# claserken/SISS

Hardware: AMD Instinct MI355X
Metric: unlearning samples/sec (= unlearning-steps/sec x batch x gpus), CelebA-HQ-256 DDPM SISS (higher is better)
Workload: dtype bf16; 1 GPU; delete_celeb.yaml: CelebA-HQ 256x256 DDPM UNet (113.7M params), SISS lambd=0.5, t=999, bf16, bs=16/GPU, GA=1, scaling_norm=500, AdamW lr 5e-6; loss_fn=importance_sampling_with_mixture, global_batch=16, grad_accum=1, parallelism=dp1, hipgraph=True

## Files before the change

### siss_amd/csrc/common.h

```cpp
#pragma once
#include <hip/hip_runtime.h>
#include <stdint.h>

typedef uint16_t bf16_t;

typedef __attribute__((ext_vector_type(8))) short bf16x8_t;
typedef __attribute__((ext_vector_type(4))) float f32x4_t;
typedef __attribute__((ext_vector_type(16))) float f32x16_t;
typedef __attribute__((ext_vector_type(4))) uint32_t u32x4_t;
typedef __attribute__((ext_vector_type(2))) uint32_t u32x2_t;
typedef __attribute__((ext_vector_type(2))) float f32x2_t;
typedef __attribute__((ext_vector_type(2))) __bf16 bf16x2_t;

#define SISS_OK 0
#define SISS_ERR_ARG 1
#define SISS_ERR_LAUNCH 2

#define SISS_CHECK_ARG(cond) \
    do {                     \
        if (!(cond)) return SISS_ERR_ARG; \
    } while (0)

#define SISS_LAUNCH_RET()                                 \
    do {                                                  \
        return hipGetLastError() == hipSuccess ? SISS_OK : SISS_ERR_LAUNCH; \
    } while (0)

__device__ __forceinline__ float bf2f(bf16_t v) {
    return __builtin_bit_cast(float, (uint32_t)v << 16);
}
__device__ __forceinline__ bf16_t f2bf(float f) {
    __bf16 b = (__bf16)f;
    return __builtin_bit_cast(bf16_t, b);
}
__device__ __forceinline__ float bfround(float f) { return bf2f(f2bf(f)); }
__device__ __forceinline__ float to_f(bf16_t v) { return bf2f(v); }
__device__ __forceinline__ float to_f(float v) { return v; }
template <typename T> __device__ __forceinline__ T from_f(float f);
template <> __device__ __forceinline__ bf16_t from_f<bf16_t>(float f) { return f2bf(f); }
template <> __device__ __forceinline__ float from_f<float>(float f) { return f; }
__device__ __forceinline__ uint32_t pack_bf2(float lo, float hi) {
    typedef float f32x2_pk __attribute__((ext_vector_type(2)));
    typedef __bf16 bf16x2_pk __attribute__((ext_vector_type(2)));
    const bf16x2_pk b = __builtin_convertvector(f32x2_pk{lo, hi}, bf16x2_pk);
    return __builtin_bit_cast(uint32_t, b);
}

__device__ __forceinline__ uint32_t add_bf16x2(uint32_t a, uint32_t b) {
    const float lo = __builtin_bit_cast(float, a << 16) + __builtin_bit_cast(float, b << 16);
    const float hi = __builtin_bit_cast(float, a & 0xffff0000u) + __builtin_bit_cast(float, b & 0xffff0000u);
    uint32_t r;
    asm("v_cvt_pk_bf16_f32 %0, %1, %2" : "=v"(r) : "v"(lo), "v"(hi));
    return r;
}

__device__ __forceinline__ float wave_sum(float v) {
#pragma unroll
    for (int o = 32; o > 0; o >>= 1) v += __shfl_xor(v, o, 64);
    return v;
}
__device__ __forceinline__ double wave_sum_d(double v) {
#pragma unroll
    for (int o = 32; o > 0; o >>= 1) v += __shfl_xor(v, o, 64);
    return v;
}

__device__ __forceinline__ float sum_lanes_mod8(float t) {
    t += __builtin_bit_cast(float, __builtin_amdgcn_update_dpp(0, __builtin_bit_cast(int, t), 0x128 , 0xf, 0xf, false));
    unsigned u = __builtin_bit_cast(unsigned, t), u2 = u;
    asm volatile("" : "+v"(u2));
    const auto a = __builtin_amdgcn_permlane16_swap(u, u2, false, false);
    unsigned a0 = a[0], a1 = a[1];
    asm volatile("" : "+v"(a0), "+v"(a1));
    t = __builtin_bit_cast(float, a0) + __builtin_bit_cast(float, a1);
    unsigned v = __builtin_bit_cast(unsigned, t), v2 = v;
    asm volatile("" : "+v"(v2));
    const auto b = __builtin_amdgcn_permlane32_swap(v, v2, false, false);
    unsigned b0 = b[0], b1 = b[1];
    asm volatile("" : "+v"(b0), "+v"(b1));
    return __builtin_bit_cast(float, b0) + __builtin_bit_cast(float, b1);
}

__device__ __forceinline__ float sigmoid_f(float z) { return __builtin_amdgcn_rcpf(1.f + __expf(-z)); }
__device__ __forceinline__ float silu_f(float z) { return z * sigmoid_f(z); }
__device__ __forceinline__ float dsilu_f(float z) {
    const float s = sigmoid_f(z);
    return s * (1.f + z * (1.f - s));
}

__device__ __forceinline__ void gelu_parts(float g, float& Phi, float& e) {
    const float x = fabsf(g) * 0.70710678118654752f;
    const float t = __builtin_amdgcn_rcpf(fmaf(0.3275911f, x, 1.f));
    e = __builtin_amdgcn_exp2f(g * g * -0.72134752044448170f);
    const float poly = t * fmaf(t, fmaf(t, fmaf(t, fmaf(t, 1.061405429f, -1.453152027f), 1.421413741f), -0.284496736f), 0.254829592f);
    const float erf_abs = fmaf(-poly, e, 1.f);
    Phi = 0.5f * (1.f + copysignf(erf_abs, g));
}
__device__ __forceinline__ float gelu_f(float g) { float P, e; gelu_parts(g, P, e); return g * P; }
__device__ __forceinline__ float dgelu_f(float g) { float P, e; gelu_parts(g, P, e); return fmaf(g * 0.3989422804014327f, e, P); }


__device__ __forceinline__ void glds16_asm(const void* g, unsigned lds_dst) {
    unsigned keep;
    asm volatile("s_mov_b32 %0, m0\n\ts_mov_b32 m0, %2\n\ts_nop 0\n\tglobal_load_lds_dwordx4 %1, off\n\ts_mov_b32 m0, %0"
                 : "=&s"(keep) : "v"(g), "s"(lds_dst) : "memory");
}
__device__ __forceinline__ void glds16_saddr(unsigned off, const void* base, unsigned lds_dst) {
    asm volatile("s_mov_b32 m0, %1\n\ts_nop 0\n\tglobal_load_lds_dwordx4 %0, %2" :: "v"(off), "s"(lds_dst), "s"(base) : "memory");
}
__device__ __forceinline__ unsigned lds_addr(const void* p) {
    return (unsigned)(size_t)(__attribute__((address_space(3))) const char*)p;
}

static inline int cdiv(long a, long b) { return (int)((a + b - 1) / b); }

constexpr int kMaxDevices = 64;
constexpr int kQsTileRows = 254, kQsHalfRows = 128;
static inline int siss_current_device() {
    int dev = 0;
    return hipGetDevice(&dev) == hipSuccess && dev >= 0 && dev < kMaxDevices ? dev : -1;
}
static inline int siss_ensure_smem(const void* kernel, int bytes, unsigned char (&done)[kMaxDevices]) {
    const int dev = siss_current_device();
    if (dev < 0) return SISS_ERR_LAUNCH;
    if (!__atomic_load_n(&done[dev], __ATOMIC_ACQUIRE)) {
        if (hipFuncSetAttribute(kernel, hipFuncAttributeMaxDynamicSharedMemorySize, bytes) != hipSuccess) return SISS_ERR_LAUNCH;
        __atomic_store_n(&done[dev], (unsigned char)1, __ATOMIC_RELEASE);
    }
    return SISS_OK;
}

enum SissKernelId { SISS_K_NT = 0, SISS_K_NT_C3P, SISS_K_FLASH_FWD, SISS_K_FLASH_BWD, SISS_K_NT_SPLITK, SISS_K_TN1, SISS_K_TN3,
                    SISS_K_GN_SLAB, SISS_K_GN_QSTATS, SISS_K_FLASH_QSPLIT, SISS_K_ATTN1H_FWD, SISS_K_ATTN1H_BWD, SISS_K_TN_PAIR, SISS_K_FLASH32, SISS_K_FLASH32_FWD, SISS_K_NT_WIDE, SISS_K_GN_SC, SISS_K_COUNT };
void siss_count_dispatch(int kernel_id);
void* siss_workspace(long* bytes);
```

### siss_amd/csrc/lora.hip

```cpp
#include "common.h"

namespace {

constexpr int kTile = 64;

struct LoraJob {
    long w_off, a_off, b_off, w0_off;
    int O, I, ptile0, mtile0;
};

template <bool MERGE>
__device__ __forceinline__ int find_job(const LoraJob* jobs, int njobs, int tile) {
    int lo = 0, hi = njobs - 1;
    while (lo < hi) {
        const int mid = (lo + hi + 1) >> 1;
        if ((MERGE ? jobs[mid].mtile0 : jobs[mid].ptile0) <= tile) lo = mid; else hi = mid - 1;
    }
    return lo;
}

constexpr f32x4_t kZero = {0.f, 0.f, 0.f, 0.f};

__device__ __forceinline__ f32x4_t ld_k4(const float* row, int k, int len, bool ok, bool vec) {
    if (!ok || k >= len) return kZero;
    if (vec) return *reinterpret_cast<const f32x4_t*>(row + k);
    f32x4_t v = kZero;
#pragma unroll
    for (int j = 0; j < 4; ++j)
        if (k + j < len) v[j] = row[k + j];
    return v;
}

template <int NT>
__global__ __launch_bounds__(256) void lora_project_kernel(const float* __restrict__ grads, long set_stride, int nsets,
                                                           const float* __restrict__ lora_p, float* __restrict__ lora_g,
                                                           long lora_set_stride, const LoraJob* __restrict__ jobs, int njobs, int r,
                                                           float s) {
    const int tile = blockIdx.x, set = blockIdx.y;
    const LoraJob jb = jobs[find_job<false>(jobs, njobs, tile)];
    const int O = jb.O, I = jb.I, lt = tile - jb.ptile0, rb = (O + kTile - 1) / kTile;
    const int lane = threadIdx.x & 63, wv = threadIdx.x >> 6, li = lane & 15, q = lane >> 4;
    const bool live = set < nsets;
    const float* dW = grads + (long)set * set_stride + jb.w_off;
    const float* A = lora_p + jb.a_off;
    const float* B = lora_p + jb.b_off;
    f32x4_t acc[NT];
#pragma unroll
    for (int n = 0; n < NT; ++n) acc[n] = kZero;

    if (lt < rb) {
        const int o0 = lt * kTile + wv * 16;
        if (o0 >= O) return;
        if (live) {
            const bool vec = (I & 3) == 0;
            const bool rok = o0 + li < O;
            const float* wrow = dW + (long)(o0 + li) * I;
            for (int k0 = 0; k0 < I; k0 += 16) {
                const int k = k0 + 4 * q;
                const f32x4_t a = ld_k4(wrow, k, I, rok, vec);
                f32x4_t b[NT];
#pragma unroll
                for (int n = 0; n < NT; ++n) b[n] = ld_k4(A + (long)(n * 16 + li) * I, k, I, n * 16 + li < r, vec);
#pragma unroll
                for (int j = 0; j < 4; ++j)
#pragma unroll
                    for (int n = 0; n < NT; ++n) acc[n] = __builtin_amdgcn_mfma_f32_16x16x4f32(a[j], b[n][j], acc[n], 0, 0, 0);
            }
        }
        float* dB = lora_g + (long)set * lora_set_stride + jb.b_off;
#pragma unroll
        for (int n = 0; n < NT; ++n)
#pragma unroll
            for (int j = 0; j < 4; ++j) {
                const int row = o0 + 4 * q + j, col = n * 16 + li;
                if (row < O && col < r) dB[(long)row * r + col] = s * acc[n][j];
            }
    } else {
        const int i0 = (lt - rb) * kTile + wv * 16;
        if (i0 >= I) return;
        const int col = i0 + li;
        const bool cok = col < I;
        if (live) {
#pragma unroll 4
            for (int o = 0; o < O; o += 4) {
                const int ko = o + q;
                const bool kok = ko < O;
                const float bv = (kok && cok) ? dW[(long)ko * I + col] : 0.f;
#pragma unroll
                for (int m = 0; m < NT; ++m) {
                    const float av = (kok && m * 16 + li < r) ? B[(long)ko * r + m * 16 + li] : 0.f;
                    acc[m] = __builtin_amdgcn_mfma_f32_16x16x4f32(av, bv, acc[m], 0, 0, 0);
                }
            }
        }
        float* dA = lora_g + (long)set * lora_set_stride + jb.a_off;
#pragma unroll
        for (int m = 0; m < NT; ++m)
#pragma unroll
            for (int j = 0; j < 4; ++j) {
                const int row = m * 16 + 4 * q + j;
                if (row < r && cok) dA[(long)row * I + col] = s * acc[m][j];
            }
    }
}

__global__ __launch_bounds__(256) void lora_merge_kernel(float* __restrict__ flat, bf16_t* __restrict__ shadow,
                                                         const float* __restrict__ w0, const float* __restrict__ lora_p,
                                                         const LoraJob* __restrict__ jobs, int njobs, int r, float s) {
    const int tile = blockIdx.x;
    const LoraJob jb = jobs[find_job<true>(jobs, njobs, tile)];
    const int O = jb.O, I = jb.I, lt = tile - jb.mtile0, cb = (I + kTile - 1) / kTile;
    const int lane = threadIdx.x & 63, wv = threadIdx.x >> 6, li = lane & 15, q = lane >> 4;
    const int o0 = (lt / cb) * kTile + wv * 16, i0 = (lt % cb) * kTile;
    if (o0 >= O) return;
    const float* A = lora_p + jb.a_off;
    const float* B = lora_p + jb.b_off;
    f32x4_t acc[4] = {kZero, kZero, kZero, kZero};
    if (s != 0.f) {
        const bool rok = o0 + li < O;
        for (int k0 = 0; k0 < r; k0 += 4) {
            const int k = k0 + q;
            const bool kok = k < r;
            const float av = (kok && rok) ? B[(long)(o0 + li) * r + k] : 0.f;
#pragma unroll
            for (int c = 0; c < 4; ++c) {
                const int col = i0 + c * 16 + li;
                const float bv = (kok && col < I) ? A[(long)k * I + col] : 0.f;
                acc[c] = __builtin_amdgcn_mfma_f32_16x16x4f32(av, bv, acc[c], 0, 0, 0);
            }
        }
    }
#pragma unroll
    for (int c = 0; c < 4; ++c)
#pragma unroll
        for (int j = 0; j < 4; ++j) {
            const int row = o0 + 4 * q + j, col = i0 + c * 16 + li;
            if (row < O && col < I) {
                const long idx = (long)row * I + col;
                const float base = w0[jb.w0_off + idx];
                const float v = s != 0.f ? fmaf(s, acc[c][j], base) : base;
                flat[jb.w_off + idx] = v;
                if (shadow) shadow[jb.w_off + idx] = f2bf(v);
            }
        }
}

}

extern "C" {

long siss_lora_tile(void) {
    return kTile;
}

int siss_lora_project(const float* grads, long set_stride, int nsets, const float* lora_p, float* lora_g, long lora_set_stride,
                      const void* jobs, int njobs, int r, float s, int total_tiles, void* stream) {
    SISS_CHECK_ARG(grads && lora_p && lora_g && jobs && njobs >= 1 && total_tiles >= njobs);
    SISS_CHECK_ARG((nsets == 1 || nsets == 2) && r >= 1 && r <= 64 && set_stride % 4 == 0 && lora_set_stride % 4 == 0);
    SISS_CHECK_ARG(((uintptr_t)grads | (uintptr_t)lora_p | (uintptr_t)lora_g) % 16 == 0);
    const dim3 grid(total_tiles, 2), block(256);
    const LoraJob* jt = static_cast<const LoraJob*>(jobs);
    hipStream_t st = (hipStream_t)stream;
#define SISS_LORA_PROJECT(NT) \
    lora_project_kernel<NT><<<grid, block, 0, st>>>(grads, set_stride, nsets, lora_p, lora_g, lora_set_stride, jt, njobs, r, s)
    switch ((r + 15) / 16) {
        case 1: SISS_LORA_PROJECT(1); break;
        case 2: SISS_LORA_PROJECT(2); break;
        case 3: SISS_LORA_PROJECT(3); break;
        default: SISS_LORA_PROJECT(4); break;
    }
#undef SISS_LORA_PROJECT
    SISS_LAUNCH_RET();
}

int siss_lora_merge(float* flat, void* shadow, const float* w0, const float* lora_p, const void* jobs, int njobs, int r, float s,
                    int total_tiles, void* stream) {
    SISS_CHECK_ARG(flat && w0 && lora_p && jobs && njobs >= 1 && total_tiles >= njobs && r >= 1 && r <= 64);
    lora_merge_kernel<<<dim3(total_tiles), dim3(256), 0, (hipStream_t)stream>>>(flat, static_cast<bf16_t*>(shadow), w0, lora_p,
                                                                                 static_cast<const LoraJob*>(jobs), njobs, r, s);
    SISS_LAUNCH_RET();
}

}
```

### siss_amd/csrc/timeemb.hip

```cpp
#include "common.h"

namespace {

constexpr int kThreads = 256;
constexpr int kMaxM = 4096;

__global__ void sincos_kernel(const int64_t* __restrict__ t, float* __restrict__ out, int B, int dim, int flip,
                              float freq_shift) {
    const int i = blockIdx.x * blockDim.x + threadIdx.x;
    const int half = dim / 2;
    if (i >= B * half) return;
    const int b = i / half, j = i - b * half;
    const float freq = expf(-logf(10000.f) * (float)j / ((float)half - freq_shift));
    const float arg = (float)t[b] * freq;
    const float s = sinf(arg), c = cosf(arg);
    float* o = out + (long)b * dim;
    if (flip) { o[j] = c; o[half + j] = s; }
    else { o[j] = s; o[half + j] = c; }
}

__global__ __launch_bounds__(kThreads) void linear_fwd_kernel(const float* __restrict__ x,
                                                              const float* __restrict__ W,
                                                              const float* __restrict__ b, float* __restrict__ y,
                                                              int M, int N, int K, int act_in) {
    const int lane = threadIdx.x & 63;
    const int n = blockIdx.x * (kThreads / 64) + (threadIdx.x >> 6);
    if (n >= N) return;
    for (int m0 = 0; m0 < M; m0 += 8) {
        float acc[8] = {};
        for (int k = lane; k < K; k += 64) {
            const float w = W[(long)n * K + k];
#pragma unroll
            for (int i = 0; i < 8; ++i) {
                if (m0 + i < M) {
                    float xv = x[(long)(m0 + i) * K + k];
                    if (act_in) xv = silu_f(xv);
                    acc[i] += xv * w;
                }
            }
        }
#pragma unroll
        for (int i = 0; i < 8; ++i) {
            const float s = wave_sum(acc[i]);
            if (lane == 0 && m0 + i < M) y[(long)(m0 + i) * N + n] = s + b[n];
        }
    }
}

__device__ __forceinline__ float dy_eff(const float* dy, const float* yact, int m, int n, int N, int Mx) {
    float d = dy[(long)m * N + n];
    if (yact) d *= dsilu_f(yact[(long)(m % Mx) * N + n]);
    return d;
}

__global__ __launch_bounds__(256) void linear_bwd_dx_kernel(const float* __restrict__ dy, const float* __restrict__ yact,
                                                            const float* __restrict__ W, float* __restrict__ dx, int M2,
                                                            int Mx, int N, int K, int accumulate) {
    __shared__ float part[4][64];
    const int m = blockIdx.y, lane = threadIdx.x & 63, w = threadIdx.x >> 6;
    const int k = blockIdx.x * 64 + lane;
    const int n0 = (int)((long)N * w / 4), n1 = (int)((long)N * (w + 1) / 4);
    float acc = 0.f;
    if (k < K)
        for (int n = n0; n < n1; ++n) acc += dy_eff(dy, yact, m, n, N, Mx) * W[(long)n * K + k];
    part[w][lane] = acc;
    __syncthreads();
    if (w == 0 && k < K) {
        const float t = part[0][lane] + part[1][lane] + part[2][lane] + part[3][lane];
        const long i = (long)m * K + k;
        dx[i] = accumulate ? dx[i] + t : t;
    }
}

__global__ void linear_bwd_dw_kernel(const float* __restrict__ dy, const float* __restrict__ yact,
                                     const float* __restrict__ x, float* __restrict__ dW, float* __restrict__ db,
                                     float* __restrict__ db2, int M2, int Mx, int set_rows, long set_stride_w, long set_stride_b, int N,
                                     int K, int act_in) {
    const long i = (long)blockIdx.x * blockDim.x + threadIdx.x;
    const int nsets = M2 / set_rows;
    if (i >= (long)nsets * N * K) return;
    const int set = i / ((long)N * K);
    const long rem = i - (long)set * N * K;
    const int n = rem / K, k = rem - (long)n * K;
    float acc = 0.f, bsum = 0.f;
    for (int j = 0; j < set_rows; ++j) {
        const int m = set * set_rows + j;
        const float d = dy_eff(dy, yact, m, n, N, Mx);
        float xv = x[(long)(m % Mx) * K + k];
        if (act_in) xv = silu_f(xv);
        acc += d * xv;
        bsum += d;
    }
    dW[(long)set * set_stride_w + (long)n * K + k] += acc;
    if (k == 0) {
        db[(long)set * set_stride_b + n] += bsum;
        if (db2) db2[(long)set * set_stride_b + n] += bsum;
    }
}


__global__ __launch_bounds__(kThreads) void multi_fwd_kernel(const float* __restrict__ x, const float* __restrict__ P,
                                                             const long* __restrict__ woff, const long* __restrict__ boff,
                                                             float* __restrict__ y, int M, int Ntot, int K) {
    const int lane = threadIdx.x & 63;
    const int n = blockIdx.x * (kThreads / 64) + (threadIdx.x >> 6);
    if (n >= Ntot) return;
    const float* W = P + woff[n];
    for (int m0 = 0; m0 < M; m0 += 8) {
        float acc[8] = {};
        for (int k = lane; k < K; k += 64) {
            const float w = W[k];
#pragma unroll
            for (int i = 0; i < 8; ++i)
                if (m0 + i < M) acc[i] += silu_f(x[(long)(m0 + i) * K + k]) * w;
        }
#pragma unroll
        for (int i = 0; i < 8; ++i) {
            const float s = wave_sum(acc[i]);
            if (lane == 0 && m0 + i < M) y[(long)(m0 + i) * Ntot + n] = s + P[boff[n]];
        }
    }
}

constexpr int kDwCols = 32, kDwRows = 32;
__global__ __launch_bounds__(256) void multi_bwd_dw_kernel(const float* __restrict__ dy, const float* __restrict__ x, float* __restrict__ G,
                                                           const long* __restrict__ woff, const long* __restrict__ boff,
                                                           const long* __restrict__ boff2, int Mx, int set_rows, long set_stride,
                                                           int Ntot, int K) {
    __shared__ float sdy[kDwRows][kDwCols + 1];
    const int k = blockIdx.x * 256 + threadIdx.x;
    const int n0 = blockIdx.y * kDwCols, set = blockIdx.z;
    const int ncols = Ntot - n0 < kDwCols ? Ntot - n0 : kDwCols;
    float acc[kDwCols];
#pragma unroll
    for (int c = 0; c < kDwCols; ++c) acc[c] = 0.f;
    float bsum = 0.f;
    for (int j0 = 0; j0 < set_rows; j0 += kDwRows) {
        const int nr = set_rows - j0 < kDwRows ? set_rows - j0 : kDwRows;
        __syncthreads();
        for (int i = threadIdx.x; i < kDwRows * kDwCols; i += 256) {
            const int r = i / kDwCols, c = i - r * kDwCols;
            sdy[r][c] = (r < nr && c < ncols) ? dy[(long)(set * set_rows + j0 + r) * Ntot + n0 + c] : 0.f;
        }
        __syncthreads();
        if (blockIdx.x == 0 && threadIdx.x < ncols)
            for (int r = 0; r < nr; ++r) bsum += sdy[r][threadIdx.x];
        if (k < K) {
            for (int r = 0; r < nr; ++r) {
                const float sx = silu_f(x[(long)((set * set_rows + j0 + r) % Mx) * K + k]);
#pragma unroll
                for (int c = 0; c < kDwCols; ++c) acc[c] += sdy[r][c] * sx;
            }
        }
    }
    float* g = G + (long)set * set_stride;
    if (k < K) {
#pragma unroll
        for (int c = 0; c < kDwCols; ++c)
            if (c < ncols) g[woff[n0 + c] + k] += acc[c];
    }
    if (blockIdx.x == 0 && threadIdx.x < ncols) {
        g[boff[n0 + threadIdx.x]] += bsum;
        g[boff2[n0 + threadIdx.x]] += bsum;
    }
}

constexpr int kDxSplit = 512;
__global__ __launch_bounds__(256) void multi_bwd_dx_kernel(const float* __restrict__ dy, const float* __restrict__ P,
                                                           const long* __restrict__ woff, float* __restrict__ dx,
                                                           int M2, int Ntot, int K) {
    const int k = blockIdx.x * 256 + threadIdx.x;
    const int m = blockIdx.y;
    const int n0 = blockIdx.z * kDxSplit;
    const int n1 = n0 + kDxSplit < Ntot ? n0 + kDxSplit : Ntot;
    if (k >= K) return;
    const float* d = dy + (long)m * Ntot;
    float a0 = 0.f, a1 = 0.f, a2 = 0.f, a3 = 0.f;
    int n = n0;
    for (; n + 4 <= n1; n += 4) {
        a0 += d[n] * P[woff[n] + k];
        a1 += d[n + 1] * P[woff[n + 1] + k];
        a2 += d[n + 2] * P[woff[n + 2] + k];
        a3 += d[n + 3] * P[woff[n + 3] + k];
    }
    for (; n < n1; ++n) a0 += d[n] * P[woff[n] + k];
    atomicAdd(dx + (long)m * K + k, (a0 + a1) + (a2 + a3));
}

}

extern "C" {

int siss_timestep_sincos(const int64_t* t, float* out, int B, int dim, int flip_sin_to_cos, float freq_shift, void* stream) {
    SISS_CHECK_ARG(t && out && B > 0 && dim > 0 && dim % 2 == 0);
    sincos_kernel<<<cdiv((long)B * dim / 2, 128), 128, 0, (hipStream_t)stream>>>(t, out, B, dim, flip_sin_to_cos, freq_shift);
    SISS_LAUNCH_RET();
}

int siss_linear_small_fwd(const float* x, const float* W, const float* b, float* y, int M, int N, int K, int act_in_silu, void* stream) {
    SISS_CHECK_ARG(x && W && b && y && M > 0 && M <= kMaxM && N > 0 && K > 0);
    linear_fwd_kernel<<<cdiv(N, kThreads / 64), kThreads, 0, (hipStream_t)stream>>>(x, W, b, y, M, N, K, act_in_silu);
    SISS_LAUNCH_RET();
}

int siss_linear_small_bwd(const float* dy, const float* yact, const float* x, const float* W, float* dx, int accumulate_dx,
                          float* dW, float* db, float* db2, int M2, int Mx, int set_rows, long set_stride_w,
                          long set_stride_b, int N, int K, int act_in_silu, void* stream) {
    SISS_CHECK_ARG(dy && x && W && dW && db && M2 > 0 && Mx > 0 && set_rows > 0 && M2 % set_rows == 0 && N > 0 && K > 0);
    hipStream_t st = (hipStream_t)stream;
    if (dx) linear_bwd_dx_kernel<<<dim3(cdiv(K, 64), M2), 256, 0, st>>>(dy, yact, W, dx, M2, Mx, N, K, accumulate_dx);
    const long tot = (long)(M2 / set_rows) * N * K;
    linear_bwd_dw_kernel<<<cdiv(tot, 256), 256, 0, st>>>(dy, yact, x, dW, db, db2, M2, Mx, set_rows, set_stride_w, set_stride_b, N, K, act_in_silu);
    SISS_LAUNCH_RET();
}

int siss_linear_multi_fwd(const float* x, const float* params, const long* woff, const long* boff, float* y, int M,
                          int Ntot, int K, void* stream) {
    SISS_CHECK_ARG(x && params && woff && boff && y && M > 0 && M <= kMaxM && Ntot > 0 && K > 0);
    multi_fwd_kernel<<<cdiv(Ntot, kThreads / 64), kThreads, 0, (hipStream_t)stream>>>(x, params, woff, boff, y, M, Ntot, K);
    SISS_LAUNCH_RET();
}

int siss_linear_multi_bwd(const float* dy, const float* x, const float* params, float* grads, const long* woff,
                          const long* boff, const long* boff2, float* dx, int M2, int Mx, int set_rows,
                          long set_stride, int Ntot, int K, void* stream) {
    SISS_CHECK_ARG(dy && x && params && grads && woff && boff && boff2 && dx);
    SISS_CHECK_ARG(M2 > 0 && M2 <= kMaxM && Mx > 0 && set_rows > 0 && M2 % set_rows == 0 && Ntot > 0 && K > 0);
    hipStream_t st = (hipStream_t)stream;
    const dim3 gw(cdiv(K, 256), cdiv(Ntot, kDwCols), M2 / set_rows);
    multi_bwd_dw_kernel<<<gw, 256, 0, st>>>(dy, x, grads, woff, boff, boff2, Mx, set_rows, set_stride, Ntot, K);
    dim3 grid(cdiv(K, 256), M2, cdiv(Ntot, kDxSplit));
    multi_bwd_dx_kernel<<<grid, 256, 0, st>>>(dy, params, woff, dx, M2, Ntot, K);
    SISS_LAUNCH_RET();
}

}
```

Before: 313.8 samples/sec.

## Use fp32 MFMA tiles for small-linear backward dW and split-N dX

Replaces the scalar per-element dW kernels for the time-embedding linears (plain and multi-table) with one templated kernel that accumulates 16x16 tiles using fp32 MFMA, loading existing gradients into the accumulators and writing them back with vector stores. The dX backward now uses an MFMA tile kernel split along N into workspace partials, followed by a separate reduce kernel, with the old kernel kept as a fallback when the workspace is too small. The aim is to cut the cost of these many small backward GEMMs. It adds a workspace dependency and an extra launch, and changes the order of floating-point summation.

```diff
diff --git a/siss_amd/csrc/common.h b/siss_amd/csrc/common.h
--- a/siss_amd/csrc/common.h
+++ b/siss_amd/csrc/common.h
@@ -81,6 +81,16 @@
     return __builtin_bit_cast(float, b0) + __builtin_bit_cast(float, b1);
 }
 
+__device__ __forceinline__ f32x4_t ld_k4(const float* row, int k, int len, bool ok, bool vec) {
+    f32x4_t v = {0.f, 0.f, 0.f, 0.f};
+    if (!ok || k >= len) return v;
+    if (vec) return *reinterpret_cast<const f32x4_t*>(row + k);
+#pragma unroll
+    for (int j = 0; j < 4; ++j)
+        if (k + j < len) v[j] = row[k + j];
+    return v;
+}
+
 __device__ __forceinline__ float sigmoid_f(float z) { return __builtin_amdgcn_rcpf(1.f + __expf(-z)); }
 __device__ __forceinline__ float silu_f(float z) { return z * sigmoid_f(z); }
 __device__ __forceinline__ float dsilu_f(float z) {
diff --git a/siss_amd/csrc/lora.hip b/siss_amd/csrc/lora.hip
--- a/siss_amd/csrc/lora.hip
+++ b/siss_amd/csrc/lora.hip
@@ -20,16 +20,6 @@
 }
 
 constexpr f32x4_t kZero = {0.f, 0.f, 0.f, 0.f};
-
-__device__ __forceinline__ f32x4_t ld_k4(const float* row, int k, int len, bool ok, bool vec) {
-    if (!ok || k >= len) return kZero;
-    if (vec) return *reinterpret_cast<const f32x4_t*>(row + k);
-    f32x4_t v = kZero;
-#pragma unroll
-    for (int j = 0; j < 4; ++j)
-        if (k + j < len) v[j] = row[k + j];
-    return v;
-}
 
 template <int NT>
 __global__ __launch_bounds__(256) void lora_project_kernel(const float* __restrict__ grads, long set_stride, int nsets,
diff --git a/siss_amd/csrc/timeemb.hip b/siss_amd/csrc/timeemb.hip
--- a/siss_amd/csrc/timeemb.hip
+++ b/siss_amd/csrc/timeemb.hip
@@ -19,6 +19,20 @@
     else { o[j] = s; o[half + j] = c; }
 }
 
+__device__ __forceinline__ bool aligned16(const void* p) { return ((uintptr_t)p & 15) == 0; }
+
+template <bool TABLE>
+__device__ __forceinline__ const float* weight_row(const float* W, const long* woff, int n, int K) {
+    return TABLE ? W + woff[n] : W + (long)n * K;
+}
+
+template <bool FAST>
+__device__ __forceinline__ f32x4_t ld_op(const float* row, int k, int len, bool ok, bool vec) {
+    if (!FAST) return ld_k4(row, k, len, ok, vec);
+    const f32x4_t v = *reinterpret_cast<const f32x4_t*>(row + (k < len ? k : 0));
+    return ok && k < len ? v : f32x4_t{0.f, 0.f, 0.f, 0.f};
+}
+
 __global__ __launch_bounds__(kThreads) void linear_fwd_kernel(const float* __restrict__ x,
                                                               const float* __restrict__ W,
                                                               const float* __restrict__ b, float* __restrict__ y,
@@ -43,6 +57,29 @@
         for (int i = 0; i < 8; ++i) {
             const float s = wave_sum(acc[i]);
             if (lane == 0 && m0 + i < M) y[(long)(m0 + i) * N + n] = s + b[n];
+        }
+    }
+}
+
+__global__ __launch_bounds__(kThreads) void multi_fwd_kernel(const float* __restrict__ x, const float* __restrict__ P,
+                                                             const long* __restrict__ woff, const long* __restrict__ boff,
+                                                             float* __restrict__ y, int M, int Ntot, int K) {
+    const int lane = threadIdx.x & 63;
+    const int n = blockIdx.x * (kThreads / 64) + (threadIdx.x >> 6);
+    if (n >= Ntot) return;
+    const float* W = P + woff[n];
+    for (int m0 = 0; m0 < M; m0 += 8) {
+        float acc[8] = {};
+        for (int k = lane; k < K; k += 64) {
+            const float w = W[k];
+#pragma unroll
+            for (int i = 0; i < 8; ++i)
+                if (m0 + i < M) acc[i] += silu_f(x[(long)(m0 + i) * K + k]) * w;
+        }
+#pragma unroll
+        for (int i = 0; i < 8; ++i) {
+            const float s = wave_sum(acc[i]);
+            if (lane == 0 && m0 + i < M) y[(long)(m0 + i) * Ntot + n] = s + P[boff[n]];
         }
     }
 }
@@ -72,97 +109,230 @@
     }
 }
 
-__global__ void linear_bwd_dw_kernel(const float* __restrict__ dy, const float* __restrict__ yact,
-                                     const float* __restrict__ x, float* __restrict__ dW, float* __restrict__ db,
-                                     float* __restrict__ db2, int M2, int Mx, int set_rows, long set_stride_w, long set_stride_b, int N,
-                                     int K, int act_in) {
-    const long i = (long)blockIdx.x * blockDim.x + threadIdx.x;
-    const int nsets = M2 / set_rows;
-    if (i >= (long)nsets * N * K) return;
-    const int set = i / ((long)N * K);
-    const long rem = i - (long)set * N * K;
-    const int n = rem / K, k = rem - (long)n * K;
-    float acc = 0.f, bsum = 0.f;
-    for (int j = 0; j < set_rows; ++j) {
-        const int m = set * set_rows + j;
-        const float d = dy_eff(dy, yact, m, n, N, Mx);
-        float xv = x[(long)(m % Mx) * K + k];
-        if (act_in) xv = silu_f(xv);
-        acc += d * xv;
-        bsum += d;
-    }
-    dW[(long)set * set_stride_w + (long)n * K + k] += acc;
-    if (k == 0) {
-        db[(long)set * set_stride_b + n] += bsum;
-        if (db2) db2[(long)set * set_stride_b + n] += bsum;
-    }
-}
-
-
-__global__ __launch_bounds__(kThreads) void multi_fwd_kernel(const float* __restrict__ x, const float* __restrict__ P,
-                                                             const long* __restrict__ woff, const long* __restrict__ boff,
-                                                             float* __restrict__ y, int M, int Ntot, int K) {
-    const int lane = threadIdx.x & 63;
-    const int n = blockIdx.x * (kThreads / 64) + (threadIdx.x >> 6);
-    if (n >= Ntot) return;
-    const float* W = P + woff[n];
-    for (int m0 = 0; m0 < M; m0 += 8) {
-        float acc[8] = {};
-        for (int k = lane; k < K; k += 64) {
-            const float w = W[k];
-#pragma unroll
-            for (int i = 0; i < 8; ++i)
-                if (m0 + i < M) acc[i] += silu_f(x[(long)(m0 + i) * K + k]) * w;
-        }
-#pragma unroll
-        for (int i = 0; i < 8; ++i) {
-            const float s = wave_sum(acc[i]);
-            if (lane == 0 && m0 + i < M) y[(long)(m0 + i) * Ntot + n] = s + P[boff[n]];
-        }
-    }
-}
-
-constexpr int kDwCols = 32, kDwRows = 32;
-__global__ __launch_bounds__(256) void multi_bwd_dw_kernel(const float* __restrict__ dy, const float* __restrict__ x, float* __restrict__ G,
-                                                           const long* __restrict__ woff, const long* __restrict__ boff,
-                                                           const long* __restrict__ boff2, int Mx, int set_rows, long set_stride,
-                                                           int Ntot, int K) {
-    __shared__ float sdy[kDwRows][kDwCols + 1];
-    const int k = blockIdx.x * 256 + threadIdx.x;
-    const int n0 = blockIdx.y * kDwCols, set = blockIdx.z;
-    const int ncols = Ntot - n0 < kDwCols ? Ntot - n0 : kDwCols;
-    float acc[kDwCols];
-#pragma unroll
-    for (int c = 0; c < kDwCols; ++c) acc[c] = 0.f;
+constexpr int kDwSub = 4;
+template <bool TABLE>
+__global__ __launch_bounds__(256, 3) void linear_bwd_dw_tile_kernel(const float* __restrict__ dy, const float* __restrict__ yact,
+                                                                 const float* __restrict__ x, float* __restrict__ dW,
+                                                                 float* __restrict__ db, float* __restrict__ db2,
+                                                                 const long* __restrict__ woff, const long* __restrict__ boff,
+                                                                 const long* __restrict__ boff2, int Mx, int set_rows,
+                                                                 long set_stride_w, long set_stride_b, int N, int K, int act_in) {
+    const int lane = threadIdx.x & 63, wv = threadIdx.x >> 6, li = lane & 15, q = lane >> 4;
+    const int n0 = blockIdx.y * 64 + 16 * wv, set = blockIdx.z;
+    if (n0 >= N) return;
+    const int k0 = blockIdx.x * (64 * kDwSub), kl = k0 + 4 * li;
+    const bool k4 = (K & 3) == 0, xvec = k4 && aligned16(x);
+    float* grow[4];
+    bool nok[4], gal = true;
+#pragma unroll
+    for (int i = 0; i < 4; ++i) {
+        const int n = n0 + 4 * q + i;
+        nok[i] = n < N;
+        const int nc = nok[i] ? n : N - 1;
+        grow[i] = dW + (long)set * set_stride_w + (TABLE ? woff[nc] : (long)nc * K);
+        gal = gal && aligned16(grow[i]);
+    }
+    const bool gfast = k4 && __all(gal);
+    f32x4_t acc[kDwSub][4];
+    if (gfast) {
+#pragma unroll
+        for (int i = 0; i < 4; ++i)
+#pragma unroll
+            for (int t = 0; t < kDwSub; ++t) {
+                const f32x4_t g = ld_op<true>(grow[i], kl + 64 * t, K, nok[i], true);
+#pragma unroll
+                for (int c = 0; c < 4; ++c) acc[t][c][i] = g[c];
+            }
+    } else {
+#pragma unroll
+        for (int t = 0; t < kDwSub; ++t)
+#pragma unroll
+            for (int c = 0; c < 4; ++c) acc[t][c] = f32x4_t{0.f, 0.f, 0.f, 0.f};
+    }
+    const bool colok = n0 + li < N;
+    const int ncol = colok ? n0 + li : N - 1;
     float bsum = 0.f;
-    for (int j0 = 0; j0 < set_rows; j0 += kDwRows) {
-        const int nr = set_rows - j0 < kDwRows ? set_rows - j0 : kDwRows;
-        __syncthreads();
-        for (int i = threadIdx.x; i < kDwRows * kDwCols; i += 256) {
-            const int r = i / kDwCols, c = i - r * kDwCols;
-            sdy[r][c] = (r < nr && c < ncols) ? dy[(long)(set * set_rows + j0 + r) * Ntot + n0 + c] : 0.f;
-        }
-        __syncthreads();
-        if (blockIdx.x == 0 && threadIdx.x < ncols)
-            for (int r = 0; r < nr; ++r) bsum += sdy[r][threadIdx.x];
-        if (k < K) {
-            for (int r = 0; r < nr; ++r) {
-                const float sx = silu_f(x[(long)((set * set_rows + j0 + r) % Mx) * K + k]);
-#pragma unroll
-                for (int c = 0; c < kDwCols; ++c) acc[c] += sdy[r][c] * sx;
+    for (int j0 = 0; j0 < set_rows; j0 += 4) {
+        const bool jok = j0 + q < set_rows;
+        const int m = set * set_rows + (jok ? j0 + q : 0), mx = m % Mx;
+        float a = dy[(long)m * N + ncol];
+        const float ya = yact ? yact[(long)mx * N + ncol] : 0.f;
+        const float* xrow = x + (long)mx * K;
+        f32x4_t bv[kDwSub];
+        if (xvec) {
+#pragma unroll
+            for (int t = 0; t < kDwSub; ++t) bv[t] = ld_op<true>(xrow, kl + 64 * t, K, jok, true);
+        } else {
+#pragma unroll
+            for (int t = 0; t < kDwSub; ++t) bv[t] = ld_k4(xrow, kl + 64 * t, K, jok, false);
+        }
+        if (yact) a *= dsilu_f(ya);
+        if (!(jok && colok)) a = 0.f;
+        bsum += a;
+        if (act_in) {
+#pragma unroll
+            for (int t = 0; t < kDwSub; ++t)
+#pragma unroll
+                for (int c = 0; c < 4; ++c) bv[t][c] = silu_f(bv[t][c]);
+        }
+#pragma unroll
+        for (int t = 0; t < kDwSub; ++t)
+#pragma unroll
+            for (int c = 0; c < 4; ++c) acc[t][c] = __builtin_amdgcn_mfma_f32_16x16x4f32(a, bv[t][c], acc[t][c], 0, 0, 0);
+    }
+#pragma unroll
+    for (int i = 0; i < 4; ++i)
+#pragma unroll
+        for (int t = 0; t < kDwSub; ++t) {
+            const int k = kl + 64 * t;
+            if (!nok[i] || k >= K) continue;
+            if (gfast) {
+                *reinterpret_cast<f32x4_t*>(grow[i] + k) = f32x4_t{acc[t][0][i], acc[t][1][i], acc[t][2][i], acc[t][3][i]};
+            } else {
+#pragma unroll
+                for (int c = 0; c < 4; ++c)
+                    if (k + c < K) grow[i][k + c] += acc[t][c][i];
             }
         }
-    }
-    float* g = G + (long)set * set_stride;
-    if (k < K) {
-#pragma unroll
-        for (int c = 0; c < kDwCols; ++c)
-            if (c < ncols) g[woff[n0 + c] + k] += acc[c];
-    }
-    if (blockIdx.x == 0 && threadIdx.x < ncols) {
-        g[boff[n0 + threadIdx.x]] += bsum;
-        g[boff2[n0 + threadIdx.x]] += bsum;
-    }
+    if (blockIdx.x == 0) {
+        bsum += __shfl_xor(bsum, 16, 64);
+        bsum += __shfl_xor(bsum, 32, 64);
+        if (q == 0 && colok) {
+            const long sb = (long)set * set_stride_b;
+            db[sb + (TABLE ? boff[ncol] : (long)ncol)] += bsum;
+            if (db2) db2[sb + (TABLE ? boff2[ncol] : (long)ncol)] += bsum;
+        }
+    }
+}
+
+
+template <bool FAST>
+__device__ __forceinline__ void dx_operands(f32x4_t (&a)[2], f32x4_t (&ya)[2], f32x4_t (&bv)[4], const float* const (&dyrow)[2],
+                                            const float* const (&yrow)[2], const bool (&rok)[2], int nq, int N,
+                                            const float* const (&wrow)[4], const bool (&nok)[4], int kl, int K, bool dvec, bool k4) {
+#pragma unroll
+    for (int g = 0; g < 2; ++g) {
+        a[g] = ld_op<FAST>(dyrow[g], nq, N, rok[g], dvec);
+        ya[g] = ld_op<FAST>(yrow[g], nq, N, rok[g], dvec);
+    }
+#pragma unroll
+    for (int j = 0; j < 4; ++j) bv[j] = ld_op<FAST>(wrow[j], kl, K, nok[j], k4 && aligned16(wrow[j]));
+}
+
+template <bool TABLE>
+__global__ __launch_bounds__(256) void linear_bwd_dx_tile_kernel(const float* __restrict__ dy, const float* __restrict__ yact,
+                                                                 const float* __restrict__ W, const long* __restrict__ woff,
+                                                                 float* __restrict__ part, int M2, int Mx, int N, int K, int Kp,
+                                                                 int chunk) {
+    __shared__ f32x4_t red[4][2][16][16];
+    const int lane = threadIdx.x & 63, wv = threadIdx.x >> 6, li = lane & 15, q = lane >> 4;
+    const int k0 = blockIdx.x * 64, kl = k0 + 4 * li;
+    const int nb = blockIdx.y * chunk, ne = nb + chunk < N ? nb + chunk : N;
+    const int mb = blockIdx.z * 32, ng = M2 - mb > 16 ? 2 : 1;
+    const bool k4 = (K & 3) == 0;
+    const bool dvec = (N & 3) == 0 && aligned16(dy) && (!yact || aligned16(yact));
+    const float *dyrow[2], *yrow[2];
+    bool rok[2];
+#pragma unroll
+    for (int g = 0; g < 2; ++g) {
+        const int m = mb + 16 * g + li;
+        rok[g] = g < ng && m < M2;
+        const int mc = m < M2 ? m : M2 - 1;
+        dyrow[g] = dy + (long)mc * N;
+        yrow[g] = yact ? yact + (long)(mc % Mx) * N : dyrow[g];
+    }
+    f32x4_t acc[2][4];
+#pragma unroll
+    for (int g = 0; g < 2; ++g)
+#pragma unroll
+        for (int c = 0; c < 4; ++c) acc[g][c] = f32x4_t{0.f, 0.f, 0.f, 0.f};
+    for (int ns = nb + 16 * wv; ns < ne; ns += 64) {
+        const int nq = ns + 4 * q;
+        const float* wrow[4];
+        bool nok[4], wal = true;
+#pragma unroll
+        for (int j = 0; j < 4; ++j) {
+            nok[j] = nq + j < N;
+            wrow[j] = weight_row<TABLE>(W, woff, nok[j] ? nq + j : N - 1, K);
+            wal = wal && aligned16(wrow[j]);
+        }
+        f32x4_t a[2], ya[2], bv[4];
+        if (dvec && k4 && __all(wal)) dx_operands<true>(a, ya, bv, dyrow, yrow, rok, nq, N, wrow, nok, kl, K, dvec, k4);
+        else dx_operands<false>(a, ya, bv, dyrow, yrow, rok, nq, N, wrow, nok, kl, K, dvec, k4);
+        if (yact) {
+#pragma unroll
+            for (int g = 0; g < 2; ++g)
+#pragma unroll
+                for (int j = 0; j < 4; ++j) a[g][j] *= dsilu_f(ya[g][j]);
+        }
+#pragma unroll
+        for (int j = 0; j < 4; ++j)
+#pragma unroll
+            for (int c = 0; c < 4; ++c) {
+                acc[0][c] = __builtin_amdgcn_mfma_f32_16x16x4f32(a[0][j], bv[j][c], acc[0][c], 0, 0, 0);
+                if (ng > 1) acc[1][c] = __builtin_amdgcn_mfma_f32_16x16x4f32(a[1][j], bv[j][c], acc[1][c], 0, 0, 0);
+            }
+    }
+#pragma unroll
+    for (int g = 0; g < 2; ++g)
+#pragma unroll
+        for (int i = 0; i < 4; ++i) red[wv][g][4 * q + i][li] = f32x4_t{acc[g][0][i], acc[g][1][i], acc[g][2][i], acc[g][3][i]};
+    __syncthreads();
+    const int row = threadIdx.x >> 4, c4 = threadIdx.x & 15;
+    for (int g = 0; g < ng; ++g) {
+        const int m = mb + 16 * g + row;
+        if (m < M2) {
+            const f32x4_t t = ((red[0][g][row][c4] + red[1][g][row][c4]) + red[2][g][row][c4]) + red[3][g][row][c4];
+            *reinterpret_cast<f32x4_t*>(part + ((long)blockIdx.y * M2 + m) * Kp + k0 + 4 * c4) = t;
+        }
+    }
+}
+
+__global__ __launch_bounds__(256) void dx_reduce_kernel(const float* __restrict__ part, float* __restrict__ dx, int S, int M2, int K,
+                                                        int Kp, int accumulate) {
+    __shared__ float fold[4][64];
+    const int lane = threadIdx.x & 63, wv = threadIdx.x >> 6;
+    const long e = (long)blockIdx.x * 64 + lane;
+    const bool ok = e < (long)M2 * K;
+    const int m = ok ? (int)(e / K) : 0, k = ok ? (int)(e - (long)m * K) : 0;
+    const int s0 = (int)((long)S * wv / 4), s1 = (int)((long)S * (wv + 1) / 4);
+    float acc = 0.f;
+    if (ok) {
+        const float* p = part + (long)m * Kp + k;
+        const long stride = (long)M2 * Kp;
+#pragma unroll 4
+        for (int s = s0; s < s1; ++s) acc += p[s * stride];
+    }
+    fold[wv][lane] = acc;
+    __syncthreads();
+    if (wv == 0 && ok) {
+        const float t = ((fold[0][lane] + fold[1][lane]) + fold[2][lane]) + fold[3][lane];
+        dx[e] = accumulate ? dx[e] + t : t;
+    }
+}
+
+bool dx_tile_plan(int M2, int N, int K, int& S, int& chunk, int& Kp, float*& ws) {
+    long bytes = 0;
+    ws = (float*)siss_workspace(&bytes);
+    if (!ws) return false;
+    bytes -= 4096;
+    const int ktiles = cdiv(K, 64);
+    Kp = ktiles * 64;
+    const long per_split = (long)M2 * Kp * (long)sizeof(float);
+    int want = cdiv(768, (long)ktiles * cdiv(M2, 32));
+    if (want < 1) want = 1;
+    chunk = cdiv(cdiv(N, want), 64) * 64;
+    while ((long)cdiv(N, chunk) * per_split > bytes && chunk < N) chunk *= 2;
+    S = cdiv(N, chunk);
+    return (long)S * per_split <= bytes;
+}
+
+template <bool TABLE>
+int launch_dx_tiles(const float* dy, const float* yact, const float* W, const long* woff, float* dx, int accumulate, int M2, int Mx,
+                    int N, int K, int S, int chunk, int Kp, float* ws, hipStream_t st) {
+    linear_bwd_dx_tile_kernel<TABLE><<<dim3(Kp / 64, S, cdiv(M2, 32)), 256, 0, st>>>(dy, yact, W, woff, ws, M2, Mx, N, K, Kp, chunk);
+    dx_reduce_kernel<<<cdiv((long)M2 * K, 64), 256, 0, st>>>(ws, dx, S, M2, K, Kp, accumulate);
+    return hipGetLastError() == hipSuccess ? SISS_OK : SISS_ERR_LAUNCH;
 }
 
 constexpr int kDxSplit = 512;
@@ -208,9 +378,17 @@
                           long set_stride_b, int N, int K, int act_in_silu, void* stream) {
     SISS_CHECK_ARG(dy && x && W && dW && db && M2 > 0 && Mx > 0 && set_rows > 0 && M2 % set_rows == 0 && N > 0 && K > 0);
     hipStream_t st = (hipStream_t)stream;
-    if (dx) linear_bwd_dx_kernel<<<dim3(cdiv(K, 64), M2), 256, 0, st>>>(dy, yact, W, dx, M2, Mx, N, K, accumulate_dx);
-    const long tot = (long)(M2 / set_rows) * N * K;
-    linear_bwd_dw_kernel<<<cdiv(tot, 256), 256, 0, st>>>(dy, yact, x, dW, db, db2, M2, Mx, set_rows, set_stride_w, set_stride_b, N, K, act_in_silu);
+    if (dx) {
+        int S, chunk, Kp;
+        float* ws;
+        if (dx_tile_plan(M2, N, K, S, chunk, Kp, ws)) {
+            if (launch_dx_tiles<false>(dy, yact, W, nullptr, dx, accumulate_dx, M2, Mx, N, K, S, chunk, Kp, ws, st) != SISS_OK) return SISS_ERR_LAUNCH;
+        } else {
+            linear_bwd_dx_kernel<<<dim3(cdiv(K, 64), M2), 256, 0, st>>>(dy, yact, W, dx, M2, Mx, N, K, accumulate_dx);
+        }
+    }
+    linear_bwd_dw_tile_kernel<false><<<dim3(cdiv(K, 64 * kDwSub), cdiv(N, 64), M2 / set_rows), 256, 0, st>>>(
+        dy, yact, x, dW, db, db2, nullptr, nullptr, nullptr, Mx, set_rows, set_stride_w, set_stride_b, N, K, act_in_silu);
     SISS_LAUNCH_RET();
 }
 
@@ -227,8 +405,12 @@
     SISS_CHECK_ARG(dy && x && params && grads && woff && boff && boff2 && dx);
     SISS_CHECK_ARG(M2 > 0 && M2 <= kMaxM && Mx > 0 && set_rows > 0 && M2 % set_rows == 0 && Ntot > 0 && K > 0);
     hipStream_t st = (hipStream_t)stream;
-    const dim3 gw(cdiv(K, 256), cdiv(Ntot, kDwCols), M2 / set_rows);
-    multi_bwd_dw_kernel<<<gw, 256, 0, st>>>(dy, x, grads, woff, boff, boff2, Mx, set_rows, set_stride, Ntot, K);
+    linear_bwd_dw_tile_kernel<true><<<dim3(cdiv(K, 64 * kDwSub), cdiv(Ntot, 64), M2 / set_rows), 256, 0, st>>>(
+        dy, nullptr, x, grads, grads, grads, woff, boff, boff2, Mx, set_rows, set_stride, set_stride, Ntot, K, 1);
+    int S, chunk, Kp;
+    float* ws;
+    if (dx_tile_plan(M2, Ntot, K, S, chunk, Kp, ws))
+        return launch_dx_tiles<true>(dy, nullptr, params, woff, dx, 1, M2, Mx, Ntot, K, S, chunk, Kp, ws, st);
     dim3 grid(cdiv(K, 256), M2, cdiv(Ntot, kDxSplit));
     multi_bwd_dx_kernel<<<grid, 256, 0, st>>>(dy, params, woff, dx, M2, Ntot, K);
     SISS_LAUNCH_RET();
```

Result: no change. 314.5 samples/sec, median of 4 (+0.2%).
